# yynps737/zero-latency-yolo

Measured on AMD Instinct MI355X. Metric: frames_per_sec, higher is better.
Workload: dtype bf16; 1 GPU; YOLOv8-nano 416x416 batch=64 throughput path (BASELINE configs[2]), bf16; engines_per_gpu=3, weights=seeded synthetic (no real weights offline), graph=True, parallelism=single GPU

## Files before the change

zero-latency-yolo_amd/csrc/engine.cpp:

```cpp
#include "zly_internal.h"
#include "weights.h"

#include <algorithm>
#include <atomic>
#include <chrono>
#include <condition_variable>
#include <deque>
#include <map>
#include <mutex>
#include <string>
#include <thread>
#include <type_traits>
#include <vector>
#include <string.h>
#include <stdio.h>
#include <stdlib.h>

namespace zly {

static thread_local std::string g_last_error;

static int fail(int code, const std::string& msg) { g_last_error = msg; return code; }

#define HIP_TRY(expr, code)                                                                        \
// ... 54 lines not shown
    size_t w1 = 0, b1 = 0, w2 = 0, b2 = 0;
    int nk1 = 0, nk2 = 0, cout2 = 0;
    int vis_of(int op) const { for (const Member& m : members) if (m.op == op) return m.vis; return 0; }
};

struct DetectTail {
    HeadArgs args{};
    int op[3] = {-1, -1, -1};
    int box[3] = {-1, -1, -1}, cls[3] = {-1, -1, -1}, logits[3] = {-1, -1, -1};
    size_t wb[3] = {}, bb[3] = {}, wc[3] = {}, bc[3] = {};
};

struct Plan {
    int nc = 0, N = 0;
    std::vector<Buffer> bufs;
    std::vector<Op> ops;
    std::vector<PairGroup> pairs;
    std::vector<C2fGroup> c2fs;
    DetectTail tail;
    int in_buf = -1;
    std::map<std::string, std::pair<int, int>> tap_index;
    std::map<std::string, std::pair<int, int>> tap_final;
    bool stem_fused = false;
    bool stem1 = false;
    size_t stem_w = 0, stem_b = 0, m1_w = 0, m1_b = 0, stem_w0p = 0;
    int stem_out = -1, m1_out = -1;
    int sppf_cv1 = -1, sppf_pool = -1, sppf_cv2 = -1;
    int det_stem[3] = {-1, -1, -1}, det_a[3] = {-1, -1, -1}, det_b[3] = {-1, -1, -1};
    bool det_merge_ok = false;
    int join_at = -1;
    std::vector<uint8_t> blob;
};

enum LaunchKind { LK_NONE, LK_PREPROCESS, LK_STEM, LK_STEM1, LK_CONV, LK_CONV_WSK, LK_MULTI, LK_C2F, LK_PAIR, LK_SPPF_FUSED, LK_SPPF_POOL, LK_HEAD, LK_NMS };
struct Launch {
    int kind = LK_NONE;
    int covered_by = -1;
    bool hbm = true;
    ConvPlan conv{};
    WskPlan wsk{};
    C2fPlan c2f{};
    PairPlan pair{};
    int multi_ct = 0;
    int only_level = -1;
    bool pool16 = false;
    bool lb = false;
};

struct Ingest;

}

using namespace zly;

struct zly_engine : Plan {
    zly_config cfg;
    std::string weights_path;
    int dev = 0;
    int dtype = ZLY_DTYPE_BF16;
    size_t esz = 2;
    ModelFile model;

    void* d_weights = nullptr;
    float* d_head = nullptr;
    Cand* d_cand = nullptr;
    Cand* d_scratch = nullptr;
    int* d_count = nullptr;
    Cand* d_cand_alt = nullptr;
    int* d_count_alt = nullptr;
    Cand* cur_cand = nullptr;
    int* cur_count = nullptr;
    hipStream_t nms_stream = nullptr;
    hipEvent_t ev_head = nullptr, ev_nms[2] = {nullptr, nullptr};
    int parity = 0;
    bool nms_recorded[2] = {false, false};
// ... 80 lines not shown
    num("ZLY_STEM1_VAR", &sw->stem1_var);
    num("ZLY_STEM1_GRID", &sw->stem1_grid);
    num("ZLY_STEM1_TW", &sw->stem1_tw);
    num("ZLY_STEM1_TH", &sw->stem1_th);
    sw->stem1_keep_tiles = on("ZLY_STEM1_TW") || on("ZLY_STEM1_TH") || on("ZLY_STEM1_BIG_TILES");
    num("ZLY_PAIR_MIN_TILES", &sw->pair_min_tiles);
    num("ZLY_PAIR_WIDTHS", &sw->pair_widths);
    auto num_nonempty = [&](const char* name, int* out) { const char* v = getenv(name); if (v && *v) *out = atoi(v); };
    num_nonempty("ZLY_STAGE_SLOTS", &sw->stage_slots);
    num_nonempty("ZLY_STAGE_MB", &sw->stage_mb);
    num_nonempty("ZLY_INFLIGHT", &sw->inflight);
    { int d = 0; num_nonempty("ZLY_D2H_STREAM", &d); sw->d2h_stream = d != 0; }
    num("ZLY_PROFILE_INNER", &sw->profile_inner);
    if (sw->profile_inner < 1) sw->profile_inner = 1;
#ifdef ZLY_DIAG
    if (const char* v = getenv("ZLY_ABLATE_SKIP")) sw->ablate = std::string(",") + v + ",";
#endif
    sw->no_stream = on("ZLY_NO_STREAM");
    sw->stream_ct2 = on("ZLY_STREAM_CT2");
    num("ZLY_STREAM_MAX_NK", &sw->stream_max_nk);
    num("ZLY_STREAM_MIN_GROUPS", &sw->stream_min_groups);
    num("ZLY_STREAM_WGS", &sw->stream_wgs);
    num("ZLY_WS1", &sw->ws1_mode);
    sw->ws1_no_dual = on("ZLY_WS1_NO_DUAL");
    num("ZLY_WS1_MIN_PX", &sw->ws1_min_px);
    sw->ws1_max_bytes = on("ZLY_WS1_MAX_BYTES");
    sw->no_ws = on("ZLY_NO_WS");
    sw->no_ws_s2 = on("ZLY_NO_WS_S2");
    sw->no_ws_s2_c32 = on("ZLY_NO_WS_S2_C32");
    sw->ws_rowt = on("ZLY_WS_ROWT");
    num("ZLY_WS_TPW1_MAXCT", &sw->ws_tpw1_maxct);
    num("ZLY_WS_MIN_TILES", &sw->ws_min_tiles);
    num("ZLY_WS_MAX_BYTES", &sw->ws_max_bytes);
    sw->no_wres = on("ZLY_NO_WRES");
    num("ZLY_WRES_MAXCHUNKS", &sw->wres_maxchunks);
    sw->lds_s2_pt1 = on("ZLY_LDS_S2_PT1");
    num("ZLY_LDS_MIN_TILES", &sw->lds_min_tiles);
    num("ZLY_LDS_WGS_PER_CU", &sw->lds_wgs_per_cu);
    num("ZLY_DIRECT_PT4_MIN", &sw->direct_pt4_min);
    num("ZLY_DIRECT_PT2_MIN", &sw->direct_pt2_min);
    num("ZLY_DIRECT_KSPLIT_NK", &sw->direct_ksplit_nk);
    num("ZLY_C2F32_NW", &sw->c2f32_nw);
    num("ZLY_C2F_LDS_KB", &sw->c2f_lds_kb);
    if (const char* ft = getenv("ZLY_C2F_TILE")) { int th = 0, tw = 0; if (sscanf(ft, "%d,%d", &th, &tw) == 2) { sw->c2f_tile_th = th; sw->c2f_tile_tw = tw; } }
    sw->c2f64 = on("ZLY_C2F64");
}

struct PlanBuilder {
    Plan* p;
    const ModelFile& model;
    const zly_config& cfg;
    const int dtype;
    const Switches& sw;
    const size_t esz;
    const int kstep;
    std::string err;

    bool bf16() const { return dtype == ZLY_DTYPE_BF16; }
    bool fail(const std::string& msg) { err = msg; return false; }
    int add_buffer(const std::string& name, int H, int W, int C, bool f32 = false) {
        Buffer b;
        b.name = name; b.H = H; b.W = W; b.C = C; b.f32 = f32;
        p->bufs.push_back(b);
        return (int)p->bufs.size() - 1;
    }
    int add_op(const Op& op) { p->ops.push_back(op); return (int)p->ops.size() - 1; }
// ... 447 lines not shown
    }
    ca.w1 = wb + g.w1; ca.b1 = (const float*)(wb + g.b1); ca.nk1 = g.nk1;
    ca.cat = cb.ptr; ca.cat_cs = cb.C; ca.pair_in_co = e->ops[(size_t)pg.first].in.co; ca.pair_out_co = pg.out.co;
    ca.wA = wb + pg.wA; ca.bA = (const float*)(wb + pg.bA); ca.wB = wb + pg.wB; ca.bB = (const float*)(wb + pg.bB);
    ca.res = g.res;
    ca.w2 = wb + g.w2; ca.b2 = (const float*)(wb + g.b2); ca.nk2 = g.nk2; ca.Cout2 = g.cout2;
    ca.out = ob.ptr; ca.out_cs = ob.C; ca.out_co = g.out.co;
    ca.H = cb.H; ca.W = cb.W; ca.n = n;
    ca.TH = pl.th; ca.TW = pl.tw; ca.tiles_x = pl.tiles_x; ca.tiles_y = pl.tiles_y; ca.total_tiles = pl.total_tiles;
    ca.dump = (e->cfg.flags & ZLY_FLAG_DUMP_LOGITS) ? 1 : 0;
    if (g.c == 64 && g.mid.buf >= 0) { const Buffer& mb = e->bufs[(size_t)g.mid.buf]; ca.mid = mb.ptr; ca.mid_cs = mb.C; }
    return ca;
}

static const std::vector<Launch>& resolve_launches(zly_engine* e, int n)
{
    auto it = e->launches.find(n);
    if (it != e->launches.end()) return it->second;
    const bool bf16 = e->dtype == ZLY_DTYPE_BF16, fusion = bf16 && !(e->cfg.flags & ZLY_FLAG_NO_FUSION), dump = (e->cfg.flags & ZLY_FLAG_DUMP_LOGITS) != 0;
    const int nops = (int)e->ops.size();
    auto c2f_of = [&](const C2fGroup& g, C2fPlan* pl) {
        if (!fusion || e->sw.no_c2f) return false;
        const Buffer& b = e->bufs[(size_t)g.cat];
        return c2f_plan(g.c, g.mode, g.nk1, g.nk2, g.cout2, n, b.H, b.W, e->sw, pl);
    };
    auto pair_of = [&](int a, PairPlan* pl) {
        const Op& A = e->ops[(size_t)a];
        if (A.pair < 0 || !fusion) return false;
        const PairGroup& g = e->pairs[(size_t)A.pair];
        if (g.first != a || !(e->sw.pair_widths & g.c)) return false;
        const Buffer& b = e->bufs[(size_t)A.in.buf];
        return pair_plan(g.c, n, b.H, b.W, e->sw, pl) && pl->total_tiles >= e->sw.pair_min_tiles;
    };
    bool sppf = fusion && e->sw.sppf_fused && e->sppf_cv1 >= 0;
    if (sppf) {
        const Op& a = e->ops[(size_t)e->sppf_cv1];
        const Op& b = e->ops[(size_t)e->sppf_cv2];
        sppf = a.act && b.act && a.res.buf < 0 && b.res.buf < 0 && a.in2.buf < 0 && b.in.C == 4 * a.cout && a.cout_pad == a.cout && b.cout_pad == b.cout &&
               sppf_fused_ok(make_sppf_args(e, n));
    }
    const bool merge = bf16 && e->det_merge_ok && n <= 4 && !lanes_active(e, n) && !e->sw.no_det_merge;
    auto merged_at = [&](int i) {
        for (int l = 0; l < 3; ++l) {
            if (i == e->det_stem[l]) return e->det_stem[2];
            if (i == e->det_a[l] || i == e->det_b[l]) return e->det_a[2];
        }
        return -1;
    };
    const bool tail_split = lanes_active(e, n) && !e->sw.no_tail_split;
    const int tail = e->tail.op[2];

    const bool lb = (e->cfg.flags & ZLY_FLAG_LETTERBOX) != 0;
    std::vector<Launch> t((size_t)nops);
    for (int i = 0; i < nops; ++i) {
        const Op& op = e->ops[(size_t)i];
        Launch& L = t[(size_t)i];
        L.covered_by = i;
        L.lb = lb && (op.kind == OP_PREPROCESS || op.kind == OP_HEAD || (i == 1 && e->stem_fused));
        auto covered = [&](int by) { L.kind = LK_NONE; L.covered_by = by; };
        switch (op.kind) {
        case OP_PREPROCESS:
            if (e->stem_fused) covered(1);
            else L.kind = LK_PREPROCESS;
            break;
        case OP_SPPF: {
            const Buffer& b = e->bufs[(size_t)op.in.buf];
            if (sppf) covered(e->sppf_cv1);
            else { L.kind = LK_SPPF_POOL; L.pool16 = sppf_pool16_ok(e->dtype, b.C, op.in.C, n, b.H, b.W, e->sw.pool_six_pass ? 1 : 0); }
            break;
        }
        case OP_HEAD:
            if (tail_split || op.level == 2) { L.kind = LK_HEAD; L.only_level = tail_split ? op.level : -1; }
            else covered(tail);
            break;
        case OP_NMS:
            L.kind = LK_NMS;
            break;
        case OP_CONV: {
            conv_plan(e->dtype, op.ks, make_conv_args(e, op, n), e->sw, &L.conv);
            C2fPlan cp{};
            PairPlan pp{};
            if (i == 1 && e->stem_fused) {
                L.kind = e->stem1 ? LK_STEM1 : LK_STEM;
                L.hbm = !e->stem1 || dump;
            } else if (i == 2 && e->stem1) {
                covered(1);
            } else if (op.c2f >= 0 && c2f_of(e->c2fs[(size_t)op.c2f], &cp)) {
                const C2fGroup& g = e->c2fs[(size_t)op.c2f];
                if (g.leader == i) { L.kind = LK_C2F; L.c2f = cp; }
                else covered(g.leader);
                L.hbm = g.vis_of(i) == 0 || (g.vis_of(i) == 1 && dump);
            } else if (sppf && i == e->sppf_cv1) {
                L.kind = LK_SPPF_FUSED;
                L.hbm = dump;
            } else if (sppf && i == e->sppf_cv2) {
                covered(e->sppf_cv1);
            } else if (merge && merged_at(i) >= 0) {
                if (merged_at(i) == i) { L.kind = LK_MULTI; L.multi_ct = i == e->det_stem[2] ? 3 : 2; }
                else covered(merged_at(i));
            } else if (pair_of(i, &pp)) {
                L.kind = LK_PAIR; L.pair = pp;
                L.hbm = false;
            } else if (op.pair >= 0 && e->pairs[(size_t)op.pair].second == i && pair_of(e->pairs[(size_t)op.pair].first, &pp)) {
                covered(e->pairs[(size_t)op.pair].first);
            } else if (op.wsk_w && !e->sw.no_wsk && bf16 && conv_wsk_ok(make_wsk_args(e, op, n), e->sw, &L.wsk)) {
                L.kind = LK_CONV_WSK;
            } else {
                L.kind = LK_CONV;
            }
            break;
        }
        }
    }
    return e->launches.emplace(n, std::move(t)).first->second;
}

struct IoView { int buf, co, C; double px, scale; };
static void op_reads(const zly_engine* e, const Op& op, std::vector<IoView>* out)
{
    if (op.kind == OP_CONV) {
        const Buffer& ib = e->bufs[(size_t)op.in.buf];
        out->push_back({op.in.buf, op.in.co, op.in.C, (double)ib.H * ib.W, op.cin_frac});
        if (op.in2.buf >= 0) { const Buffer& b2 = e->bufs[(size_t)op.in2.buf]; out->push_back({op.in2.buf, op.in2.co, op.in2.C, (double)b2.H * b2.W, op.cin_frac}); }
        if (op.res.buf >= 0) { const Buffer& rb = e->bufs[(size_t)op.res.buf]; out->push_back({op.res.buf, op.res.co, op.res.C > 0 ? op.res.C : op.cout, (double)rb.H * rb.W, 1.0}); }
    } else if (op.kind == OP_SPPF) {
        const Buffer& b = e->bufs[(size_t)op.in.buf];
        out->push_back({op.in.buf, op.in.co, op.in.C, (double)b.H * b.W, 1.0});
    } else if (op.kind == OP_HEAD) {
        const int box = e->tail.box[op.level], cls = e->tail.cls[op.level];
        const Buffer& bb = e->bufs[(size_t)box];
        const Buffer& cb = e->bufs[(size_t)cls];
        out->push_back({box, 0, bb.C, (double)bb.H * bb.W, 1.0});
        out->push_back({cls, 0, cb.C, (double)cb.H * cb.W, 1.0});
    }
}
static void op_writes(const zly_engine* e, const Op& op, std::vector<IoView>* out)
{
// ... 16 lines not shown
    case LK_NONE:
        return hipSuccess;
    case LK_PREPROCESS:
        return launch_preprocess(e->dtype, d_src, e->d_desc, n, e->bufs[(size_t)e->in_buf].ptr, nullptr, e->cfg.model_w, e->cfg.model_h, s, e->front_yuv, L.lb, e->front_view);
    case LK_STEM: {
        StemArgs st = e->stem;
        st.src = d_src; st.desc = e->d_desc;
        return launch_stem_fused(st, n, s, e->front_yuv, L.lb, e->front_view);
    }
    case LK_STEM1: {
        Stem1Args st = e->stem1a;
        st.st.src = d_src; st.st.desc = e->d_desc;
        return launch_stem_model1(st, n, s, e->front_yuv, L.lb, e->front_view);
    }
    case LK_CONV:
        return launch_conv(make_conv_args(e, op, n), L.conv, s);
    case LK_CONV_WSK:
        return launch_conv_wsk(make_wsk_args(e, op, n), L.wsk, s);
    case LK_MULTI: {
        ConvArgsMulti m{};
        for (int l = 0; l < 3; ++l) {
            if (L.multi_ct == 3) m.a[m.n++] = make_conv_args(e, e->ops[(size_t)e->det_stem[l]], n);
            else { m.a[m.n++] = make_conv_args(e, e->ops[(size_t)e->det_a[l]], n); m.a[m.n++] = make_conv_args(e, e->ops[(size_t)e->det_b[l]], n); }
        }
        return launch_conv_multi(m, L.multi_ct, s);
    }
    case LK_C2F: {
        const C2fGroup& g = e->c2fs[(size_t)op.c2f];
        return launch_c2f(g.c, g.mode, make_c2f_args(e, g, L.c2f, n), L.c2f, s);
    }
    case LK_PAIR: {
        const PairGroup& g = e->pairs[(size_t)op.pair];
        return launch_pair(g.c, make_pair_args(e, g, L.pair, n), L.pair, s);
    }
    case LK_SPPF_FUSED:
        return launch_sppf_fused(make_sppf_args(e, n), s);
    case LK_SPPF_POOL: {
        const Buffer& b = e->bufs[(size_t)op.in.buf];
        return launch_sppf_pool(e->dtype, b.ptr, b.C, op.in.C, n, b.H, b.W, s, e->sw.pool_six_pass ? 1 : 0);
    }
    case LK_HEAD: {
        HeadArgs h = e->tail.args;
        h.only_level = L.only_level;
        if (L.lb) { h.lb_tw = e->cfg.model_w; h.lb_th = e->cfg.model_h; }
        h.head = (e->cfg.flags & ZLY_FLAG_NO_HEAD_TENSOR) ? nullptr : e->d_head; h.desc = e->d_desc; h.conf_thr = e->cfg.conf_thr; h.cand = e->cur_cand; h.cand_count = e->cur_count;
        return launch_head_fused(e->dtype, h, n, s);
    }
    case LK_NMS:
        return launch_nms(e->cur_cand, e->cur_count, e->N, n, e->cfg.iou_thr, e->nc, e->d_scratch,
                          d_slabs_out ? d_slabs_out : e->d_slabs, e->cfg.max_dets, tag0, s, e->sw.nms_general ? 1 : 0);
    }
    return hipErrorInvalidValue;
}

static hipError_t run_ops(zly_engine* e, const std::vector<Launch>& tab, size_t first, size_t last, int n, hipStream_t s)
{
    bool forked[3] = {false, false, false};
    hipError_t r = hipSuccess;
    auto join_all = [&]() {
        for (int l = 1; l <= 2 && r == hipSuccess; ++l) {
            if (!forked[l]) continue;
            r = hipEventRecord(e->ev_join[l - 1], e->side[l - 1]);
            if (r == hipSuccess) r = hipStreamWaitEvent(s, e->ev_join[l - 1], 0);
            forked[l] = false;
        }
    };
// ... 1336 lines not shown
    if (n_candidates) *n_candidates = hd->n_candidates;
    return ZLY_OK;
}

int32_t zly_debug_tap(zly_engine* e, const char* name, int32_t idx, float* out, size_t cap_floats, int32_t* c, int32_t* h, int32_t* w)
{
    if (!e) return fail(ZLY_ERR_NOT_INITIALIZED, "Engine not running");
    if (!name || !out || idx < 0 || idx >= e->cfg.max_batch) return fail(ZLY_ERR_INVALID_ARGUMENT, "bad argument");
    std::lock_guard<std::mutex> lk(e->mu);
    ExclusiveGate gl;
    HIP_TRY(hipSetDevice(e->dev), ZLY_ERR_SYSTEM);
    int buf = -1, co = 0, C = 0;
    bool f32 = false;
    if (std::string(name) == "images") { buf = e->in_buf; co = 0; C = 3; }
    else {
        auto it = e->tap_index.find(name);
        auto jt = e->tap_final.find(name);
        if (it != e->tap_index.end()) {
            const Op& op = e->ops[(size_t)it->second.first];
            const std::vector<Launch>* t = e->last_n > 0 ? &resolve_launches(e, e->last_n) : nullptr;
            const Launch* L = t ? &(*t)[(size_t)it->second.first] : nullptr;
            switch (L && !L->hbm ? (*t)[(size_t)L->covered_by].kind : LK_NONE) {
            case LK_STEM1:
                if (e->last_front)
                    return fail(ZLY_ERR_INVALID_ARGUMENT, "tap model.0 stays in LDS inside the fused stem kernel; create the engine with ZLY_FLAG_DUMP_LOGITS (or ZLY_FLAG_NO_FUSION)");
                break;
            case LK_C2F:
                return fail(ZLY_ERR_INVALID_ARGUMENT, std::string("tap ") + name + " stays in LDS inside the fused C2f kernel at this batch size; create the engine with " +
                                                          (e->c2fs[(size_t)op.c2f].vis_of(it->second.first) == 1 ? "ZLY_FLAG_DUMP_LOGITS or " : "") + "ZLY_FLAG_NO_FUSION");
            case LK_SPPF_FUSED:
                return fail(ZLY_ERR_INVALID_ARGUMENT, std::string("tap ") + name + " stays in LDS inside the fused SPPF kernel; create the engine with ZLY_FLAG_DUMP_LOGITS or ZLY_FLAG_NO_FUSION");
            case LK_PAIR:
                return fail(ZLY_ERR_INVALID_ARGUMENT, std::string("tap ") + name + " stays in LDS inside the fused bottleneck kernel at this batch size; create the engine with ZLY_FLAG_NO_FUSION");
            }
            buf = op.out.buf; co = op.out.co + op.tap_co[(size_t)it->second.second]; C = op.tap_c[(size_t)it->second.second];
            f32 = op.out_f32 != 0;
        } else if (jt != e->tap_final.end()) {
            if (!(e->cfg.flags & ZLY_FLAG_DUMP_LOGITS))
                return fail(ZLY_ERR_INVALID_ARGUMENT, std::string("tap ") + name + " is computed inside the fused Detect kernel; create the engine with ZLY_FLAG_DUMP_LOGITS");
            buf = jt->second.first; co = jt->second.second; C = co == 0 ? 64 : e->nc; f32 = true;
        } else {
            return fail(ZLY_ERR_INVALID_ARGUMENT, std::string("unknown tap: ") + name);
        }
    }
    const Buffer& b = e->bufs[(size_t)buf];
    const size_t elems = (size_t)C * b.H * b.W;
    if (elems > cap_floats) return fail(ZLY_ERR_INVALID_ARGUMENT, "tap output buffer too small");
    int rc = ensure_scratch_f32(e, elems);
    if (rc != ZLY_OK) return rc;
    HIP_TRY(launch_tap_to_nchw(f32 ? ZLY_DTYPE_FP32 : e->dtype, b.ptr, b.C, co, C, b.H, b.W, idx, e->d_scratch_f32, e->stream), ZLY_ERR_INFERENCE);
    HIP_TRY(hipMemcpyAsync(out, e->d_scratch_f32, elems * sizeof(float), hipMemcpyDeviceToHost, e->stream), ZLY_ERR_INFERENCE);
    HIP_TRY(hipStreamSynchronize(e->stream), ZLY_ERR_INFERENCE);
    if (c) *c = C;
    if (h) *h = b.H;
    if (w) *w = b.W;
    return ZLY_OK;
}

int32_t zly_num_classes(const zly_engine* e) { return e ? e->nc : 0; }
int32_t zly_weights_fp8(const zly_engine* e) { return (e && e->model.fp8_weights) ? 1 : 0; }
int32_t zly_num_anchors(const zly_engine* e) { return e ? e->N : 0; }
int32_t zly_num_ops(const zly_engine* e) { return e ? (int32_t)e->ops.size() : 0; }

int32_t zly_op_info_at(const zly_engine* e, int32_t i, zly_op_info* out)
{
    if (!e || !out || i < 0 || i >= (int32_t)e->ops.size()) return fail(ZLY_ERR_INVALID_ARGUMENT, "bad argument");
    const Op& op = e->ops[(size_t)i];
    memset(out, 0, sizeof *out);
    snprintf(out->name, sizeof out->name, "%s", op.name.c_str());
    out->kind = op.kind;
    out->flops_per_frame = op.flops;
    out->bytes_per_frame = op.bytes;
    return ZLY_OK;
}

int32_t zly_op_kernel_name(zly_engine* e, int32_t i, int32_t n, char* out, size_t cap)
{
    if (!e || !out || cap < 8 || i < 0 || i >= (int32_t)e->ops.size() || n < 1 || n > e->cfg.max_batch) return fail(ZLY_ERR_INVALID_ARGUMENT, "bad argument");
    std::lock_guard<std::mutex> lk(e->mu);
    const std::vector<Launch>& t = resolve_launches(e, n);
    const Launch& L = t[(size_t)i];
    const Op& op = e->ops[(size_t)i];
    std::string k;
    switch (L.kind) {
    case LK_NONE:
        switch (t[(size_t)L.covered_by].kind) {
        case LK_STEM: case LK_STEM1: k = op.kind == OP_PREPROCESS ? "(fused into stem_fused_kernel)" : "(fused into the previous launch)"; break;
        case LK_PAIR: k = "(fused into the previous launch)"; break;
        case LK_C2F: k = "(fused into the C2f kernel at " + e->ops[(size_t)L.covered_by].name + ")"; break;
        case LK_SPPF_FUSED: k = "(fused into the SPPF kernel at model.9.cv1)"; break;
        case LK_MULTI: k = "(in a merged Detect launch)"; break;
        case LK_HEAD: k = "(covered by the last tail launch)"; break;
        }
        break;
    case LK_PREPROCESS: k = L.lb ? "preprocess_kernel<LB> (letterbox)" : "preprocess_kernel"; break;
    case LK_STEM: k = L.lb ? "stem_fused_kernel<LB> (letterbox)" : "stem_fused_kernel"; break;
    case LK_STEM1: k = L.lb ? "stem_model1_kernel<LB> (letterbox preprocess+model.0+model.1)" : "stem_model1_kernel (preprocess+model.0+model.1)"; break;
    case LK_SPPF_POOL: k = L.pool16 ? "sppf_pool16_kernel<DPP row windows, one barrier>" : "sppf_pool_kernel"; break;
    case LK_SPPF_FUSED: k = "sppf_fused_kernel<cv1+3 pools+cv2,SPLIT=" + std::to_string(sppf_split(e->ops[(size_t)e->sppf_cv2].cout, n, e->sw)) + ">"; break;
    case LK_MULTI: k = L.multi_ct == 3 ? "conv_igemm_multi_kernel<CT=3> (the 3 Detect stems)" : "conv_igemm_multi_kernel<CT=2> (the 6 Detect branch convs)"; break;
    case LK_C2F: {
        const C2fGroup& g = e->c2fs[(size_t)op.c2f];
        k = "c2f_kernel<C=" + std::to_string(g.c) + (g.c == 32 ? ",NW=" + std::to_string(L.c2f.nw) : std::string()) +
            (g.mode == 3 ? ",cv1+bottleneck+cv2>" : g.mode == 1 ? ",cv1+bottleneck>" : ",bottleneck+cv2>");
        break;
    }
    case LK_PAIR: k = "bottleneck_pair_kernel<" + std::to_string(e->pairs[(size_t)op.pair].c) + ">"; break;
    case LK_CONV_WSK: k = "conv3x3_wsk_kernel<K=720 packed across taps,5 channel tiles>"; break;
    case LK_CONV: {
        const int cin = op.in.C + (op.in2.buf >= 0 ? op.in2.C : 0);
        const ConvPlan& c = L.conv;
        switch (c.kind) {
        case CONV_WS1: k = std::string("conv1x1_ws_kernel<") + (op.in2.buf >= 0 ? "dual-source," : "") + "NK=" + std::to_string(cin / 32) + "," + std::to_string(c.ct) + " channel tiles," + std::to_string(c.pt * 16) + " px>"; break;
        case CONV_WS: k = std::string("conv3x3_ws_kernel<") + (op.stride == 2 ? "S=2," : "") + (c.rowt ? "ROWT," : "") + (c.tpw1 ? "TPW=1," : "TPW=2,") + std::to_string(c.ct) + " channel tiles>"; break;
        case CONV_LDS: k = "conv3x3_lds_kernel<S=" + std::to_string(op.stride) + ",CT=" + std::to_string(c.ct) + ",PT=" + std::to_string(c.pt) + (c.wres ? ",wres>" : ">"); break;
        case CONV_STREAM: k = "conv1x1_stream_kernel<CT=" + std::to_string(c.ct) + ",PT=" + std::to_string(c.pt) + ",NK=" + std::to_string((cin + 31) / 32) + ">"; break;
        default: k = std::string("conv_igemm_kernel<") + (op.ks == 1 ? (op.in2.buf >= 0 ? "1x1 dual-source" : "1x1") : (c.fastk ? "3x3" : "3x3 generic-K")) +
                 ",CT=" + std::to_string(c.ct) + ",PT=" + std::to_string(c.pt) + ",KSPLIT=" + std::to_string(c.ksplit) + ">";
        }
        break;
    }
    case LK_HEAD: k = L.lb ? "head_fused_kernel<LB> (letterbox box mapping)" : "head_fused_kernel"; break;
    case LK_NMS: k = "nms_kernel"; break;
    }
    snprintf(out, cap, "%s", k.c_str());
    return ZLY_OK;
}

int32_t zly_launch_info_at(zly_engine* e, int32_t i, int32_t n, zly_launch_info* out)
{
    if (!e || !out || i < 0 || i >= (int32_t)e->ops.size() || n < 1 || n > e->cfg.max_batch) return fail(ZLY_ERR_INVALID_ARGUMENT, "bad argument");
    std::lock_guard<std::mutex> lk(e->mu);
    memset(out, 0, sizeof *out);
    const int nops = (int)e->ops.size();
    const std::vector<Launch>& t = resolve_launches(e, n);
    out->covered_by = t[(size_t)i].covered_by;
    if (out->covered_by != i) return ZLY_OK;
    std::vector<char> in_group((size_t)nops, 0);
    for (int j = 0; j < nops; ++j) in_group[(size_t)j] = t[(size_t)j].covered_by == i ? 1 : 0;
    std::map<int, std::vector<char>> written_in, read_out, counted_in, counted_out;
// ... 113 lines not shown
```

zero-latency-yolo_amd/csrc/kernels_conv.hip:

```cpp
#include "zly_internal.h"
#include "conv_device.h"
#include <type_traits>
#include <algorithm>

namespace zly {

template <int CT>
__device__ __forceinline__ void load_bias(const ConvArgs& a, int tile0, int kq, f32x4 (&bias)[CT])
{
    const int ntiles = (a.Cout + 15) >> 4;
    const int paired = (ntiles >> 1) << 1;
#pragma unroll
    for (int c = 0; c < CT; ++c) {
        const int ch = tile_channel(tile0 + c, kq, paired);
        bias[c] = ch < a.Cout ? *reinterpret_cast<const f32x4*>(a.bias + ch) : f32x4{0.f, 0.f, 0.f, 0.f};
    }
}

template <typename T, int CT>
__device__ __forceinline__ void epilogue_px(const ConvArgs& a, f32x4 (&v)[CT], const f32x4 (&bias)[CT], int tile0, int kq, int m)
{
    const int ntiles = (a.Cout + 15) >> 4;
    const int paired = (ntiles >> 1) << 1;
    f32x4 o[CT];
// ... 913 lines not shown
            pair_mma(pxa, acca);
            for (int t0 = wp + 2 * g.nwp; t0 < nct; t0 += 2 * g.nwp) {
                const unsigned char* pxb[2];
                int obb[2], rbb[2];
                f32x4 accb[2][TPW];
                pair_setup(t0, pxb, obb, rbb);
                pair_store(acca, oba, rba);
                pair_mma(pxb, accb);
#pragma unroll
                for (int h2 = 0; h2 < 2; ++h2) {
                    oba[h2] = obb[h2]; rba[h2] = rbb[h2];
#pragma unroll
                    for (int c = 0; c < TPW; ++c) acca[h2][c] = accb[h2][c];
                }
            }
            pair_store(acca, oba, rba);
        }
        WSPHASE(2);
        if (tl + (int)gridDim.x < g.total_tiles) {
            __syncthreads();
            dma_patch(tl + gridDim.x, lpatch);
        }
        WSPHASE(1);
    }
#ifdef ZLY_WS_DIAG
    if (lane == 0 && g_ws_diag) {
        unsigned long long* o = g_ws_diag + ((size_t)blockIdx.x * (blockDim.x >> 6) + wave) * 8;
        for (int k = 0; k < 3; ++k) o[k] = dsum[k];
        o[3] = __builtin_amdgcn_s_memtime() - dstart;
    }
#endif
}

template <int NKS>
__global__ __launch_bounds__(320, 3) void conv3x3_wsk_kernel(const ConvArgs a, const WsGeom g)
{
    extern __shared__ __attribute__((aligned(16))) unsigned char smem[];
    unsigned char* lpatch = smem;
    const int PW = g.TW + 8, PH = g.TH + 2, PWV = g.TW + 2;
    const int tid = threadIdx.x, lane = tid & 63;
    const int wave = __builtin_amdgcn_readfirstlane(tid >> 6);
    const int nwaves = blockDim.x >> 6;
    const int p = lane & 15, kq = lane >> 4;
    const bf16_t* __restrict__ in = static_cast<const bf16_t*>(a.in) + a.in_co;
    const int upp = a.Cin >> 3;
    const float invPW = 1.0f / (float)PW, invTW = 1.0f / (float)g.TW;
    const int NPB = g.TH * g.TW, nct = (NPB + 15) >> 4;
    const int tiles_per_img = g.tiles_x * g.tiles_y;
    const int ntiles_c = (a.Cout + 15) >> 4;
    const int tile = min(wave, ntiles_c - 1);

    bf16x8 w[NKS];
    {
        const bf16_t* __restrict__ wb = static_cast<const bf16_t*>(a.wgt) + lane * 8;
#pragma unroll
        for (int s = 0; s < NKS; ++s) w[s] = *reinterpret_cast<const bf16x8*>(wb + ((size_t)tile * a.nk + s) * 512);
    }
    const int ch0 = tile * 16 + kq * 4;
    const f32x4 biasr = ch0 < a.Cout ? *reinterpret_cast<const f32x4*>(a.bias + ch0) : f32x4{0.f, 0.f, 0.f, 0.f};
    const __amdgpu_buffer_rsrc_t rout = __builtin_amdgcn_make_buffer_rsrc(a.out, 0, (unsigned)((size_t)a.M * a.out_cs * 2), 0x00020000);
    unsigned toff2[(NKS + 1) / 2];
#pragma unroll
    for (int s2 = 0; s2 < (NKS + 1) / 2; ++s2) {
        unsigned v = 0;
#pragma unroll
        for (int h = 0; h < 2; ++h) {
// ... 150 lines not shown
{
    if (stride == 2) {
        if (res || rowt) return nullptr;
        if (tpw == 1) return cin == 64 ? conv3x3_ws_kernel<1, 18, false, false, 2> : nullptr;
        if (tpw != 2) return nullptr;
        return cin == 64 ? conv3x3_ws_kernel<2, 18, false, false, 2> : cin == 32 ? conv3x3_ws_kernel<2, 9, false, false, 2> : nullptr;
    }
    if (cin != 64) return nullptr;
    if (rowt && tpw == 2) return res ? conv3x3_ws_kernel<2, 18, true, true> : conv3x3_ws_kernel<2, 18, false, true>;
    if (res) return tpw == 2 ? conv3x3_ws_kernel<2, 18, true> : conv3x3_ws_kernel<1, 18, true>;
    return tpw == 2 ? conv3x3_ws_kernel<2, 18, false> : conv3x3_ws_kernel<1, 18, false>;
}
static constexpr int WS_LDS_MAX = 64 * 1024;

static bool ws_plan(int H, int W, int cin, int n, int ncu, WsGeom* g, int stride = 1)
{
    if (!pick_ws(cin, 2, false, false, stride)) return false;
    const int pitch = cin * 2 + (stride == 2 ? 16 : 32);
    long best = -1;
    for (int th = (stride == 2 ? 2 : 4); th <= 32; ++th)
        for (int tw = 8; tw <= 32; ++tw) {
            const long ph = stride == 2 ? 2 * th + 1 : th + 2, pw = stride == 2 ? tw + 8 * ((tw + 8) / 8) : tw + 8;
            const long lds = (ph * pw * pitch + 1023) / 1024 * 1024;
            if (lds > WS_LDS_MAX) continue;
            const int tx = (W + tw - 1) / tw, ty = (H + th - 1) / th;
            const long tiles = (long)tx * ty * n;
            const long rounds = (tiles + 2 * ncu - 1) / (2 * ncu);
            const long key = rounds * ((th * tw + 15) / 16 * 16 + 64) * 4096 + ph * pw;
            if (best < 0 || key < best) { best = key; g->TH = th; g->TW = tw; g->tiles_x = tx; g->tiles_y = ty; }
        }
    if (best < 0) return false;
    g->pitch = pitch; g->nchunks = cin / 32;
    return true;
}

hipError_t ws_init()
{
    {
        hipError_t r = hipFuncSetAttribute((const void*)conv3x3_wsk_kernel<23>, hipFuncAttributeMaxDynamicSharedMemorySize, WS_LDS_MAX);
        if (r != hipSuccess) return r;
    }
    for (int tpw = 1; tpw <= 2; ++tpw)
        for (int res = 0; res <= 1; ++res)
            for (int rowt = 0; rowt <= 1; ++rowt) {
                hipError_t r = hipFuncSetAttribute((const void*)pick_ws(64, tpw, res != 0, rowt != 0), hipFuncAttributeMaxDynamicSharedMemorySize, WS_LDS_MAX);
                if (r != hipSuccess) return r;
            }
    for (int cin = 32; cin <= 64; cin += 32) {
        hipError_t r = hipFuncSetAttribute((const void*)pick_ws(cin, 2, false, false, 2), hipFuncAttributeMaxDynamicSharedMemorySize, WS_LDS_MAX);
        if (r != hipSuccess) return r;
    }
    {
        hipError_t r = hipFuncSetAttribute((const void*)pick_ws(64, 1, false, false, 2), hipFuncAttributeMaxDynamicSharedMemorySize, WS_LDS_MAX);
        if (r != hipSuccess) return r;
    }
    return hipSuccess;
}

template <int TPW, int NK, bool DUAL = false>
__global__ __launch_bounds__(256, 2) void conv1x1_ws_kernel(const ConvArgs a, const Ws1Geom g)
{
    extern __shared__ __attribute__((aligned(16))) unsigned char smem[];
    const int tid = threadIdx.x, lane = tid & 63;
    const int wave = __builtin_amdgcn_readfirstlane(tid >> 6);
    const int p = lane & 15, kq = lane >> 4;
    const int wc = wave % g.nwc, wp = wave / g.nwc;
// ... 500 lines not shown
```

zero-latency-yolo_amd/csrc/zly_internal.h:

```cpp
#pragma once
#include <hip/hip_runtime.h>
#include <stdint.h>
#include <stddef.h>
#include <string>
#include "zly.h"

namespace zly {

typedef __bf16 bf16_t;

struct FrameDesc {
    unsigned long long src_off;
    int w, h;
};
#define ZLY_DESC_FMT_SHIFT 56
__host__ __device__ __forceinline__ unsigned long long desc_pack(unsigned long long off, int fmt) { return off | ((unsigned long long)fmt << ZLY_DESC_FMT_SHIFT); }
__host__ __device__ __forceinline__ unsigned long long desc_off(unsigned long long v) { return v & ((1ull << ZLY_DESC_FMT_SHIFT) - 1); }
__host__ __device__ __forceinline__ int desc_fmt(unsigned long long v) { return (int)(v >> ZLY_DESC_FMT_SHIFT); }

struct ViewRec {
    unsigned long long off1, off2;
    int pitch0, pitch1, pitch2;
    int pad_;
};
// ... 37 lines not shown
    bool nms_general = false;
    bool no_cout_pad = false;
    bool no_cin_pad = false;
    bool no_stem1 = false;
    int  stem1_nw = 0;
    int  stem1_var = 1;
    int  stem1_grid = 0;
    int  stem1_tw = 0, stem1_th = 0;
    bool stem1_keep_tiles = false;
    int  pair_min_tiles = 32;
    int  pair_widths = 48;
    int  stage_slots = 6;
    int  stage_mb = 0;
    int  inflight = 2;
    bool d2h_stream = false;
    int  profile_inner = 1;
    std::string ablate;
    bool no_stream = false;
    bool stream_ct2 = false;
    int  stream_max_nk = 1 << 30;
    long stream_min_groups = 4096;
    int  stream_wgs = 0;
    int  ws1_mode = 1;
    bool ws1_no_dual = false;
    long ws1_min_px = 2048;
    bool ws1_max_bytes = false;
    bool no_ws = false;
    bool no_ws_s2 = false;
    bool no_ws_s2_c32 = false;
    bool ws_rowt = false;
    int  ws_tpw1_maxct = 6;
    long ws_min_tiles = 64;
    size_t ws_max_bytes = (size_t)1 << 31;
    bool no_wres = false;
    int  wres_maxchunks = 1;
    bool lds_s2_pt1 = false;
    long lds_min_tiles = 384;
    int  lds_wgs_per_cu = 0;
    long direct_pt4_min = 1024, direct_pt2_min = 512;
    int  direct_ksplit_nk = 1 << 30;
    int  c2f32_nw = 0;
    int  c2f_lds_kb = 0;
    int  c2f_tile_th = 0, c2f_tile_tw = 0;
    bool c2f64 = false;
};

enum ConvKind { CONV_DIRECT, CONV_LDS, CONV_STREAM, CONV_WS, CONV_WS1 };
struct WsGeom { int TH, TW, tiles_x, tiles_y, total_tiles, pitch, nchunks, nwc, nwp; };
struct Ws1Geom { int npx, total_tiles, pitch, nwc, nwp; };
struct ConvPlan {
    int kind;
    int ct, pt, ksplit;
    int fastk;
    int wres, rowt, tpw1;
    const void* fn[2];
    unsigned gx, gy;
    unsigned lds;
    int tiles_x, tiles_per_img, total_tiles;
    int ngroups;
    int tiles0;
    WsGeom ws;
    Ws1Geom ws1;
};
void       conv_plan(int dtype, int ks, const ConvArgs& a, const Switches& sw, ConvPlan* plan);
hipError_t launch_conv(const ConvArgs& a, const ConvPlan& plan, hipStream_t s);
hipError_t conv_init();
struct WskPlan { WsGeom g; unsigned gx, lds; };
bool       conv_wsk_ok(const ConvArgs& a, const Switches& sw, WskPlan* plan);
hipError_t launch_conv_wsk(const ConvArgs& a, const WskPlan& plan, hipStream_t s);
int        conv_kstep(int dtype);

struct PairArgs {
    const void* in;  int in_cs, in_co;
    void* out;       int out_cs, out_co;
    const void* wA;  const float* bA;
    const void* wB;  const float* bB;
    int H, W, n;
    int TH, TW, tiles_x, tiles_y, total_tiles;
    int res;
};
struct PairPlan { int th, tw, tiles_x, tiles_y, total_tiles, grid, lds_bytes; };
bool       pair_plan(int c, int n, int H, int W, const Switches& sw, PairPlan* plan);
hipError_t pair_init();
hipError_t launch_pair(int c, const PairArgs& a, const PairPlan& plan, hipStream_t s);

struct C2fArgs {
    const void* x;  int x_cs, x_co;
    const void* x2; int x2_cs, x2_co, split_c;
    const void* w1; const float* b1; int nk1;
    void* cat; int cat_cs;
    int pair_in_co, pair_out_co;
    const void* wA; const float* bA; const void* wB; const float* bB; int res;
    const void* w2; const float* b2; int nk2, Cout2;
    void* out; int out_cs, out_co;
    int H, W, n;
    int TH, TW, tiles_x, tiles_y, total_tiles;
    int dump;
    void* mid; int mid_cs;
};
struct C2fPlan { int th, tw, tiles_x, tiles_y, total_tiles, grid, lds_bytes, nw; };
bool       c2f_plan(int c, int mode, int nk1, int nk2, int cout2, int n, int H, int W, const Switches& sw, C2fPlan* plan);
hipError_t c2f_init();
hipError_t launch_c2f(int c, int mode, const C2fArgs& a, const C2fPlan& plan, hipStream_t s);
// ... 88 lines not shown
```

Before: 110,300 frames/s.

## Fuse 64-channel bottleneck conv pairs into one weight-stationary kernel with LDS intermediate

Adds a conv3x3_ws_pair_kernel that runs both 3x3 convolutions of a 64-channel bottleneck in one launch. The intermediate activation (with halo) stays in LDS, and both weight sets are held in registers. Each block walks persistent tiles and prefetches the next input patch by DMA while the second conv runs. This removes the HBM round-trip of the intermediate and one launch per bottleneck, at the cost of recomputing the halo and carrying higher register and LDS pressure. It only applies when both convs would already use the weight-stationary path and the tile count is small.

```diff
diff --git a/zero-latency-yolo_amd/csrc/engine.cpp b/zero-latency-yolo_amd/csrc/engine.cpp
--- a/zero-latency-yolo_amd/csrc/engine.cpp
+++ b/zero-latency-yolo_amd/csrc/engine.cpp
@@ -110,7 +110,7 @@
     std::vector<uint8_t> blob;
 };
 
-enum LaunchKind { LK_NONE, LK_PREPROCESS, LK_STEM, LK_STEM1, LK_CONV, LK_CONV_WSK, LK_MULTI, LK_C2F, LK_PAIR, LK_SPPF_FUSED, LK_SPPF_POOL, LK_HEAD, LK_NMS };
+enum LaunchKind { LK_NONE, LK_PREPROCESS, LK_STEM, LK_STEM1, LK_CONV, LK_CONV_WSK, LK_MULTI, LK_C2F, LK_PAIR, LK_WS_PAIR, LK_SPPF_FUSED, LK_SPPF_POOL, LK_HEAD, LK_NMS };
 struct Launch {
     int kind = LK_NONE;
     int covered_by = -1;
@@ -119,6 +119,7 @@
     WskPlan wsk{};
     C2fPlan c2f{};
     PairPlan pair{};
+    WsPairPlan ws_pair{};
     int multi_ct = 0;
     int only_level = -1;
     bool pool16 = false;
@@ -265,6 +266,9 @@
     num("ZLY_WS_TPW1_MAXCT", &sw->ws_tpw1_maxct);
     num("ZLY_WS_MIN_TILES", &sw->ws_min_tiles);
     num("ZLY_WS_MAX_BYTES", &sw->ws_max_bytes);
+    num("ZLY_WS_PAIR", &sw->ws_pair);
+    num("ZLY_WS_PAIR_GRID", &sw->ws_pair_grid);
+    num("ZLY_WS_PAIR_MAX_TILES", &sw->ws_pair_max_tiles);
     sw->no_wres = on("ZLY_NO_WRES");
     num("ZLY_WRES_MAXCHUNKS", &sw->wres_maxchunks);
     sw->lds_s2_pt1 = on("ZLY_LDS_S2_PT1");
@@ -778,6 +782,17 @@
         const Buffer& b = e->bufs[(size_t)A.in.buf];
         return pair_plan(g.c, n, b.H, b.W, e->sw, pl) && pl->total_tiles >= e->sw.pair_min_tiles;
     };
+    auto ws_pair_of = [&](int a, WsPairPlan* pl) {
+        const Op& A = e->ops[(size_t)a];
+        if (A.pair < 0 || !fusion) return false;
+        const PairGroup& g = e->pairs[(size_t)A.pair];
+        if (g.first != a || g.c != 64 || (e->sw.pair_widths & 64)) return false;
+        const ConvArgs ca = make_conv_args(e, A, n), cb = make_conv_args(e, e->ops[(size_t)g.second], n);
+        ConvPlan pa{}, pb{};
+        conv_plan(e->dtype, 3, ca, e->sw, &pa);
+        conv_plan(e->dtype, 3, cb, e->sw, &pb);
+        return conv_ws_pair_plan(ca, cb, pa, pb, e->sw, pl);
+    };
     bool sppf = fusion && e->sw.sppf_fused && e->sppf_cv1 >= 0;
     if (sppf) {
         const Op& a = e->ops[(size_t)e->sppf_cv1];
@@ -826,6 +841,7 @@
             conv_plan(e->dtype, op.ks, make_conv_args(e, op, n), e->sw, &L.conv);
             C2fPlan cp{};
             PairPlan pp{};
+            WsPairPlan wp{};
             if (i == 1 && e->stem_fused) {
                 L.kind = e->stem1 ? LK_STEM1 : LK_STEM;
                 L.hbm = !e->stem1 || dump;
@@ -849,6 +865,11 @@
                 L.hbm = false;
             } else if (op.pair >= 0 && e->pairs[(size_t)op.pair].second == i && pair_of(e->pairs[(size_t)op.pair].first, &pp)) {
                 covered(e->pairs[(size_t)op.pair].first);
+            } else if (ws_pair_of(i, &wp)) {
+                L.kind = LK_WS_PAIR; L.ws_pair = wp;
+                L.hbm = dump;
+            } else if (op.pair >= 0 && e->pairs[(size_t)op.pair].second == i && ws_pair_of(e->pairs[(size_t)op.pair].first, &wp)) {
+                covered(e->pairs[(size_t)op.pair].first);
             } else if (op.wsk_w && !e->sw.no_wsk && bf16 && conv_wsk_ok(make_wsk_args(e, op, n), e->sw, &L.wsk)) {
                 L.kind = LK_CONV_WSK;
             } else {
@@ -931,6 +952,10 @@
     case LK_PAIR: {
         const PairGroup& g = e->pairs[(size_t)op.pair];
         return launch_pair(g.c, make_pair_args(e, g, L.pair, n), L.pair, s);
+    }
+    case LK_WS_PAIR: {
+        const PairGroup& g = e->pairs[(size_t)op.pair];
+        return launch_conv_ws_pair(make_conv_args(e, op, n), make_conv_args(e, e->ops[(size_t)g.second], n), L.ws_pair, (e->cfg.flags & ZLY_FLAG_DUMP_LOGITS) != 0, s);
     }
     case LK_SPPF_FUSED:
         return launch_sppf_fused(make_sppf_args(e, n), s);
@@ -2333,6 +2358,8 @@
                 return fail(ZLY_ERR_INVALID_ARGUMENT, std::string("tap ") + name + " stays in LDS inside the fused SPPF kernel; create the engine with ZLY_FLAG_DUMP_LOGITS or ZLY_FLAG_NO_FUSION");
             case LK_PAIR:
                 return fail(ZLY_ERR_INVALID_ARGUMENT, std::string("tap ") + name + " stays in LDS inside the fused bottleneck kernel at this batch size; create the engine with ZLY_FLAG_NO_FUSION");
+            case LK_WS_PAIR:
+                return fail(ZLY_ERR_INVALID_ARGUMENT, std::string("tap ") + name + " stays in LDS inside the fused bottleneck kernel at this batch size; create the engine with ZLY_FLAG_DUMP_LOGITS or ZLY_FLAG_NO_FUSION");
             }
             buf = op.out.buf; co = op.out.co + op.tap_co[(size_t)it->second.second]; C = op.tap_c[(size_t)it->second.second];
             f32 = op.out_f32 != 0;
@@ -2387,7 +2414,7 @@
     case LK_NONE:
         switch (t[(size_t)L.covered_by].kind) {
         case LK_STEM: case LK_STEM1: k = op.kind == OP_PREPROCESS ? "(fused into stem_fused_kernel)" : "(fused into the previous launch)"; break;
-        case LK_PAIR: k = "(fused into the previous launch)"; break;
+        case LK_PAIR: case LK_WS_PAIR: k = "(fused into the previous launch)"; break;
         case LK_C2F: k = "(fused into the C2f kernel at " + e->ops[(size_t)L.covered_by].name + ")"; break;
         case LK_SPPF_FUSED: k = "(fused into the SPPF kernel at model.9.cv1)"; break;
         case LK_MULTI: k = "(in a merged Detect launch)"; break;
@@ -2407,6 +2434,7 @@
         break;
     }
     case LK_PAIR: k = "bottleneck_pair_kernel<" + std::to_string(e->pairs[(size_t)op.pair].c) + ">"; break;
+    case LK_WS_PAIR: k = std::string("conv3x3_ws_pair_kernel<") + (e->pairs[(size_t)op.pair].res ? "RES," : "") + "64->64->64," + std::to_string(L.ws_pair.g.TH) + "x" + std::to_string(L.ws_pair.g.TW) + " tiles>"; break;
     case LK_CONV_WSK: k = "conv3x3_wsk_kernel<K=720 packed across taps,5 channel tiles>"; break;
     case LK_CONV: {
         const int cin = op.in.C + (op.in2.buf >= 0 ? op.in2.C : 0);
diff --git a/zero-latency-yolo_amd/csrc/kernels_conv.hip b/zero-latency-yolo_amd/csrc/kernels_conv.hip
--- a/zero-latency-yolo_amd/csrc/kernels_conv.hip
+++ b/zero-latency-yolo_amd/csrc/kernels_conv.hip
@@ -969,6 +969,229 @@
 #endif
 }
 
+__device__ __forceinline__ void ws_pair_mma(const bf16x8 (&w)[18], const unsigned char* const (&px)[2], const int (&toff)[18], f32x4 (&acc)[2])
+{
+    constexpr int WS_DEPTH = 3;
+    acc[0] = f32x4{0.f, 0.f, 0.f, 0.f};
+    acc[1] = f32x4{0.f, 0.f, 0.f, 0.f};
+    bf16x8 xf[2][WS_DEPTH + 1];
+#pragma unroll
+    for (int s = 0; s < WS_DEPTH; ++s) { xf[0][s] = *reinterpret_cast<const bf16x8*>(px[0] + toff[s]); xf[1][s] = *reinterpret_cast<const bf16x8*>(px[1] + toff[s]); }
+#pragma unroll
+    for (int s = 0; s < 18; ++s) {
+        if (s + WS_DEPTH < 18) {
+            xf[0][(s + WS_DEPTH) % (WS_DEPTH + 1)] = *reinterpret_cast<const bf16x8*>(px[0] + toff[s + WS_DEPTH]);
+            xf[1][(s + WS_DEPTH) % (WS_DEPTH + 1)] = *reinterpret_cast<const bf16x8*>(px[1] + toff[s + WS_DEPTH]);
+        }
+        acc[0] = mma_step(w[s], xf[0][s % (WS_DEPTH + 1)], acc[0]);
+        acc[1] = mma_step(w[s], xf[1][s % (WS_DEPTH + 1)], acc[1]);
+    }
+}
+
+constexpr int WS_PAIR_PATCH_MAX = 32 * 1024, WS_PAIR_MID_MAX = 32 * 1024;
+
+template <bool RES>
+__global__ __launch_bounds__(256, 2) void conv3x3_ws_pair_kernel(const WsPairArgs a, const WsPairGeom g)
+{
+    __shared__ __attribute__((aligned(16))) unsigned char lpatch[WS_PAIR_PATCH_MAX];
+    __shared__ __attribute__((aligned(16))) unsigned char lmid[WS_PAIR_MID_MAX];
+    constexpr int NKS = 18, PITCH = 160, UPITCH = PITCH / 16, UPP = 8;
+    typedef __attribute__((ext_vector_type(2))) unsigned int u32x2;
+    const int PWA = g.TW + 4, PHA = g.TH + 4;
+    const int MW = g.TW + 8, NRT = g.TH + 2;
+    const int tid = threadIdx.x, lane = tid & 63;
+    const int wave = __builtin_amdgcn_readfirstlane(tid >> 6);
+    const int p = lane & 15, kq = lane >> 4;
+    const int ch0 = tile_channel(wave, kq, 4);
+    const int NPB = g.TH * g.TW, nct = (NPB + 15) >> 4;
+    const int tiles_per_img = g.tiles_x * g.tiles_y;
+    const float invPWA = 1.0f / (float)PWA, invTW = 1.0f / (float)g.TW, inv_upitch = 1.0f / (float)UPITCH;
+    const bf16_t* __restrict__ in = static_cast<const bf16_t*>(a.in) + a.in_co;
+    const __amdgpu_buffer_rsrc_t rin = __builtin_amdgcn_make_buffer_rsrc(const_cast<bf16_t*>(in), 0, (unsigned)(((size_t)a.n * a.H * a.W * a.in_cs - a.in_co) * 2), 0x00020000);
+    const unsigned npx = (unsigned)((size_t)a.n * a.H * a.W);
+    const __amdgpu_buffer_rsrc_t rout = __builtin_amdgcn_make_buffer_rsrc(a.out, 0, npx * (unsigned)a.out_cs * 2, 0x00020000);
+    const __amdgpu_buffer_rsrc_t rres = __builtin_amdgcn_make_buffer_rsrc(const_cast<void*>(a.res ? a.res : a.out), 0, npx * (unsigned)(a.res ? a.res_cs : a.out_cs) * 2, 0x00020000);
+    const __amdgpu_buffer_rsrc_t rmid = __builtin_amdgcn_make_buffer_rsrc(a.mid ? a.mid : a.out, 0, npx * (unsigned)(a.mid ? a.mid_cs : a.out_cs) * 2, 0x00020000);
+    const bool dump = a.mid != nullptr;
+
+    const int NLU = PHA * PWA * UPITCH, ndma = (NLU + 63) >> 6;
+    auto dma_patch = [&](int tl) {
+        const int b = tl / tiles_per_img;
+        const int r = tl - b * tiles_per_img;
+        const int ty = r / g.tiles_x;
+        const int y0 = ty * g.TH, x0 = (r - ty * g.tiles_x) * g.TW;
+        for (int k = wave; k < ndma; k += 4) {
+            const int u = k * 64 + lane;
+            const int px = (int)(((float)u + 0.5f) * inv_upitch), part = u - px * UPITCH;
+            const int py = (int)(((float)px + 0.5f) * invPWA), pxx = px - py * PWA;
+            const int gy = y0 - 2 + py, gx = x0 - 2 + pxx;
+            const bool ok = part < UPP && py < PHA && (unsigned)gy < (unsigned)a.H && (unsigned)gx < (unsigned)a.W;
+            const unsigned off = ok ? (unsigned)((((b * a.H + gy) * a.W + gx) * a.in_cs) * 2 + part * 16) : 0x80000000u;
+            __builtin_amdgcn_raw_ptr_buffer_load_lds(rin, (__attribute__((address_space(3))) void*)(lpatch + k * 1024), 16, off, 0, 0, 0);
+        }
+    };
+    if ((int)blockIdx.x < g.total_tiles) dma_patch(blockIdx.x);
+    asm volatile("" ::: "memory");
+    __builtin_amdgcn_sched_barrier(0);
+
+    const f32x4 biasA = *reinterpret_cast<const f32x4*>(a.bA + ch0);
+    bf16x8 wA[NKS], wB[NKS];
+    {
+        const bf16_t* __restrict__ wb = static_cast<const bf16_t*>(a.wA) + (size_t)wave * NKS * 512 + lane * 8;
+#pragma unroll
+        for (int s = 0; s < NKS; ++s) wA[s] = *reinterpret_cast<const bf16x8*>(wb + s * 512);
+    }
+    asm volatile("" ::: "memory");
+    __builtin_amdgcn_sched_barrier(0);
+    {
+        const bf16_t* __restrict__ wb = static_cast<const bf16_t*>(a.wB) + (size_t)wave * NKS * 512 + lane * 8;
+#pragma unroll
+        for (int s = 0; s < NKS; ++s) wB[s] = *reinterpret_cast<const bf16x8*>(wb + s * 512);
+    }
+    asm volatile("" ::: "memory");
+    __builtin_amdgcn_sched_barrier(0);
+
+    int toffA[NKS], toffB[NKS];
+#pragma unroll
+    for (int s = 0; s < NKS; ++s) {
+        const int tap = s >> 1, chunk = s & 1;
+        const int ky = tap / 3, kx = tap - ky * 3;
+        toffA[s] = (ky * PWA + kx) * PITCH + chunk * 64;
+        toffB[s] = (ky * MW + kx) * PITCH + chunk * 64;
+    }
+
+#ifdef ZLY_WS_DIAG
+    unsigned long long dsum[4] = {0, 0, 0, 0}, dT0 = 0, dT1 = 0;
+    const unsigned long long dstart = __builtin_amdgcn_s_memtime();
+    WSSTAMP(dT0);
+#endif
+    bool first = true;
+    for (int tl = blockIdx.x; tl < g.total_tiles; tl += gridDim.x) {
+        const int b = tl / tiles_per_img;
+        const int r = tl - b * tiles_per_img;
+        const int ty = r / g.tiles_x;
+        const int y0 = ty * g.TH, x0 = (r - ty * g.tiles_x) * g.TW;
+        f32x4 biasB = *reinterpret_cast<const f32x4*>(a.bB + ch0);
+        asm volatile("" ::: "memory");
+        __builtin_amdgcn_sched_barrier(0);
+        if (first) asm volatile("s_waitcnt vmcnt(19)" ::: "memory");
+        else       asm volatile("s_waitcnt vmcnt(0)" ::: "memory");
+        first = false;
+        __syncthreads();
+        WSPHASE(0);
+
+        {
+            auto setup = [&](int t0, const unsigned char* (&px)[2], int (&lo)[2], unsigned (&msk)[2], int (&db)[2]) {
+#pragma unroll
+                for (int h2 = 0; h2 < 2; ++h2) {
+                    const int rr = min(t0 + h2, NRT - 1);
+                    px[h2] = lpatch + (rr * PWA + p) * PITCH + kq * 16;
+                    lo[h2] = (rr * MW + p) * PITCH + ch0 * 2;
+                    const int gy = y0 - 1 + rr, gx = x0 - 1 + p;
+                    const bool inside = (unsigned)gy < (unsigned)a.H && (unsigned)gx < (unsigned)a.W;
+                    msk[h2] = inside ? 0xffffffffu : 0u;
+                    const bool interior = inside && rr >= 1 && rr <= g.TH && p >= 1 && p <= g.TW;
+                    db[h2] = interior ? (((b * a.H + gy) * a.W + gx) * a.mid_cs + a.mid_co + ch0) * 2 : (int)0x80000000;
+                }
+            };
+            auto store = [&](const f32x4 (&acc)[2], const int (&lo)[2], const unsigned (&msk)[2], const int (&db)[2]) {
+#pragma unroll
+                for (int h2 = 0; h2 < 2; ++h2) {
+                    f32x4 o = acc[h2] + biasA;
+#pragma unroll
+                    for (int k = 0; k < 4; ++k) o[k] = silu<bf16_t>(o[k]);
+                    u32x2 bits = __builtin_bit_cast(u32x2, to_bf16x4(o));
+                    bits[0] &= msk[h2]; bits[1] &= msk[h2];
+                    *reinterpret_cast<u32x2*>(lmid + lo[h2]) = bits;
+                    if (dump) __builtin_amdgcn_raw_buffer_store_b64(bits, rmid, db[h2], 0, 0);
+                }
+            };
+            const unsigned char* pxa[2];
+            int loa[2], dba[2];
+            unsigned mka[2];
+            f32x4 acca[2];
+            setup(0, pxa, loa, mka, dba);
+            ws_pair_mma(wA, pxa, toffA, acca);
+            for (int t0 = 2; t0 < NRT; t0 += 2) {
+                const unsigned char* pxb[2];
+                int lob[2], dbb[2];
+                unsigned mkb[2];
+                f32x4 accb[2];
+                setup(t0, pxb, lob, mkb, dbb);
+                store(acca, loa, mka, dba);
+                ws_pair_mma(wA, pxb, toffA, accb);
+#pragma unroll
+                for (int h2 = 0; h2 < 2; ++h2) { loa[h2] = lob[h2]; mka[h2] = mkb[h2]; dba[h2] = dbb[h2]; acca[h2] = accb[h2]; }
+            }
+            store(acca, loa, mka, dba);
+        }
+        WSPHASE(1);
+        __syncthreads();
+#pragma unroll
+        for (int s = 0; s < NKS; ++s) asm volatile("" : "+v"(wB[s]));
+        asm volatile("" : "+v"(biasB));
+        if (tl + (int)gridDim.x < g.total_tiles) dma_patch(tl + gridDim.x);
+        WSPHASE(2);
+
+        {
+            auto setup = [&](int t0, const unsigned char* (&px)[2], int (&ob)[2], int (&rb)[2]) {
+#pragma unroll
+                for (int h2 = 0; h2 < 2; ++h2) {
+                    const int t = min(t0 + h2, nct - 1);
+                    const int q = t * 16 + p;
+                    const int qc = min(q, NPB - 1);
+                    const int oy = (int)(((float)qc + 0.5f) * invTW), ox = qc - oy * g.TW;
+                    px[h2] = lmid + (oy * MW + ox) * PITCH + kq * 16;
+                    const int gy = y0 + oy, gx = x0 + ox;
+                    const bool ok = (t0 + h2 < nct) && q < NPB && gy < a.H && gx < a.W;
+                    const int m = (b * a.H + gy) * a.W + gx;
+                    ob[h2] = ok ? (m * a.out_cs + a.out_co + ch0) * 2 : (int)0x80000000;
+                    rb[h2] = ok ? (m * a.res_cs + a.res_co + ch0) * 2 : (int)0x80000000;
+                }
+            };
+            auto store = [&](const f32x4 (&acc)[2], const int (&ob)[2], const int (&rb)[2]) {
+#pragma unroll
+                for (int h2 = 0; h2 < 2; ++h2) {
+                    f32x4 o = acc[h2] + biasB;
+#pragma unroll
+                    for (int k = 0; k < 4; ++k) o[k] = silu<bf16_t>(o[k]);
+                    f32x4 x = o;
+                    if (RES) {
+                        const bf16x4 rv = __builtin_bit_cast(bf16x4, __builtin_amdgcn_raw_buffer_load_b64(rres, rb[h2], 0, 0));
+                        x += f32x4{(float)rv[0], (float)rv[1], (float)rv[2], (float)rv[3]};
+                    }
+                    const bf16x4 wv = to_bf16x4(x);
+                    __builtin_amdgcn_raw_buffer_store_b64(__builtin_bit_cast(u32x2, wv), rout, ob[h2], 0, 0);
+                }
+            };
+            const unsigned char* pxa[2];
+            int oba[2], rba[2];
+            f32x4 acca[2];
+            setup(0, pxa, oba, rba);
+            ws_pair_mma(wB, pxa, toffB, acca);
+            for (int t0 = 2; t0 < nct; t0 += 2) {
+                const unsigned char* pxb[2];
+                int obb[2], rbb[2];
+                f32x4 accb[2];
+                setup(t0, pxb, obb, rbb);
+                store(acca, oba, rba);
+                ws_pair_mma(wB, pxb, toffB, accb);
+#pragma unroll
+                for (int h2 = 0; h2 < 2; ++h2) { oba[h2] = obb[h2]; rba[h2] = rbb[h2]; acca[h2] = accb[h2]; }
+            }
+            store(acca, oba, rba);
+        }
+        WSPHASE(3);
+    }
+#ifdef ZLY_WS_DIAG
+    if (lane == 0 && g_ws_diag) {
+        unsigned long long* o = g_ws_diag + ((size_t)blockIdx.x * 4 + wave) * 8;
+        for (int k = 0; k < 4; ++k) o[k] = dsum[k];
+        o[4] = __builtin_amdgcn_s_memtime() - dstart;
+    }
+#endif
+}
+
 template <int NKS>
 __global__ __launch_bounds__(320, 3) void conv3x3_wsk_kernel(const ConvArgs a, const WsGeom g)
 {
@@ -1185,6 +1408,60 @@
     if (best < 0) return false;
     g->pitch = pitch; g->nchunks = cin / 32;
     return true;
+}
+
+static bool ws_pair_tiles(int H, int W, int n, int ncu, WsPairGeom* g, unsigned* lds)
+{
+    long best = -1;
+    for (int th = 4; th <= 32; ++th)
+        for (int tw = 8; tw <= 14; ++tw) {
+            const long patch = ((long)(th + 4) * (tw + 4) * 160 + 1023) / 1024 * 1024, mid = (long)(th + 2) * (tw + 8) * 160;
+            if (patch + 1024 > WS_PAIR_PATCH_MAX || mid > WS_PAIR_MID_MAX) continue;
+            const int tx = (W + tw - 1) / tw, ty = (H + th - 1) / th;
+            const long tiles = (long)tx * ty * n;
+            const long rounds = (tiles + 2 * ncu - 1) / (2 * ncu);
+            const long key = rounds * ((th + 2) * 16 + (th * tw + 15) / 16 * 16 + 64) * 65536 + patch + mid;
+            if (best < 0 || key < best) { best = key; g->TH = th; g->TW = tw; g->tiles_x = tx; g->tiles_y = ty; *lds = (unsigned)(WS_PAIR_PATCH_MAX + WS_PAIR_MID_MAX); }
+        }
+    return best >= 0;
+}
+
+typedef void (*conv_ws_pair_fn)(const WsPairArgs, const WsPairGeom);
+
+bool conv_ws_pair_plan(const ConvArgs& a, const ConvArgs& b, const ConvPlan& pa, const ConvPlan& pb, const Switches& sw, WsPairPlan* plan)
+{
+    if (!sw.ws_pair || pa.kind != CONV_WS || pb.kind != CONV_WS) return false;
+    if (pa.rowt || pb.rowt) return false;
+    if (a.Cin != 64 || a.Cout != 64 || a.cout_pad != 64 || a.nk != 18 || b.Cin != 64 || b.Cout != 64 || b.cout_pad != 64 || b.nk != 18) return false;
+    if (a.stride != 1 || b.stride != 1 || a.pad != 1 || b.pad != 1 || !a.act || !b.act || a.res || a.in2 || b.in2 || a.out_f32 || b.out_f32) return false;
+    if (a.H != a.Ho || a.W != a.Wo || b.H != a.H || b.W != a.W || b.Ho != a.H || b.Wo != a.W || a.M != b.M) return false;
+    if (b.in != a.out || b.in_cs != a.out_cs || b.in_co != a.out_co) return false;
+    if (a.out_cs % 4 || a.out_co % 4 || b.out_cs % 4 || b.out_co % 4 || (b.res && (b.res_cs % 4 || b.res_co % 4))) return false;
+    const int n = a.M / (a.Ho * a.Wo);
+    WsPairPlan p{};
+    if (!ws_pair_tiles(a.H, a.W, n, sw.num_cus, &p.g, &p.lds)) return false;
+    p.g.total_tiles = p.g.tiles_x * p.g.tiles_y * n;
+    if (p.g.total_tiles > (long)sw.ws_pair_max_tiles * 2 * sw.num_cus) return false;
+    int gx = p.g.total_tiles < 2 * sw.num_cus ? p.g.total_tiles : 2 * sw.num_cus;
+    if (sw.ws_pair_grid > 0 && gx > sw.ws_pair_grid) gx = sw.ws_pair_grid;
+    p.gx = (unsigned)gx;
+    p.fn = b.res ? (const void*)conv3x3_ws_pair_kernel<true> : (const void*)conv3x3_ws_pair_kernel<false>;
+    *plan = p;
+    return true;
+}
+
+hipError_t launch_conv_ws_pair(const ConvArgs& a, const ConvArgs& b, const WsPairPlan& plan, bool dump, hipStream_t s)
+{
+    if (!plan.fn || plan.gx < 1) return hipErrorInvalidValue;
+    WsPairArgs pa{};
+    pa.in = a.in; pa.in_cs = a.in_cs; pa.in_co = a.in_co;
+    pa.wA = a.wgt; pa.bA = a.bias; pa.wB = b.wgt; pa.bB = b.bias;
+    pa.H = a.H; pa.W = a.W; pa.n = a.M / (a.Ho * a.Wo);
+    pa.out = b.out; pa.out_cs = b.out_cs; pa.out_co = b.out_co;
+    pa.res = b.res; pa.res_cs = b.res_cs; pa.res_co = b.res_co;
+    if (dump) { pa.mid = a.out; pa.mid_cs = a.out_cs; pa.mid_co = a.out_co; }
+    hipLaunchKernelGGL(reinterpret_cast<conv_ws_pair_fn>(const_cast<void*>(plan.fn)), dim3(plan.gx), dim3(256), 0, s, pa, plan.g);
+    return hipGetLastError();
 }
 
 hipError_t ws_init()
diff --git a/zero-latency-yolo_amd/csrc/zly_internal.h b/zero-latency-yolo_amd/csrc/zly_internal.h
--- a/zero-latency-yolo_amd/csrc/zly_internal.h
+++ b/zero-latency-yolo_amd/csrc/zly_internal.h
@@ -93,6 +93,9 @@
     int  ws_tpw1_maxct = 6;
     long ws_min_tiles = 64;
     size_t ws_max_bytes = (size_t)1 << 31;
+    int  ws_pair = 1;
+    int  ws_pair_max_tiles = 2;
+    int  ws_pair_grid = 0;
     bool no_wres = false;
     int  wres_maxchunks = 1;
     bool lds_s2_pt1 = false;
@@ -130,6 +133,19 @@
 bool       conv_wsk_ok(const ConvArgs& a, const Switches& sw, WskPlan* plan);
 hipError_t launch_conv_wsk(const ConvArgs& a, const WskPlan& plan, hipStream_t s);
 int        conv_kstep(int dtype);
+struct WsPairArgs {
+    const void* in;  int in_cs, in_co;
+    const void* wA;  const float* bA;
+    const void* wB;  const float* bB;
+    int H, W, n;
+    void* out;       int out_cs, out_co;
+    const void* res; int res_cs, res_co;
+    void* mid;       int mid_cs, mid_co;
+};
+struct WsPairGeom { int TH, TW, tiles_x, tiles_y, total_tiles; };
+struct WsPairPlan { WsPairGeom g; unsigned gx, lds; const void* fn; };
+bool       conv_ws_pair_plan(const ConvArgs& a, const ConvArgs& b, const ConvPlan& pa, const ConvPlan& pb, const Switches& sw, WsPairPlan* plan);
+hipError_t launch_conv_ws_pair(const ConvArgs& a, const ConvArgs& b, const WsPairPlan& plan, bool dump, hipStream_t s);
 
 struct PairArgs {
     const void* in;  int in_cs, in_co;
```

After: 111,400 frames/s (median of 6 runs). 1.01x the previous value.
